# codelion/adaptive-classifier

Measured on NVIDIA H100. Metric: queries/sec predict() bert-base 128-tok, 1M x 768 prototypes, higher is better.
Workload: dtype f16

## Files before the change

### adaptive_classifier_b200/csrc/common.cuh

```cuda
#pragma once

#include <cuda_runtime.h>
#include <cuda.h>
#include <stdint.h>
#include <stdio.h>
#include <string.h>
#include <string>

#include "../../include/adaptive_b200.h"

namespace ac {

void set_error(const char *fmt, ...);
int check_cuda(cudaError_t e, const char *what);

#define AC_CUDA(call)                                                \
    do {                                                             \
        int _rc = ::ac::check_cuda((call), #call);                   \
        if (_rc != 0) return _rc;                                    \
    } while (0)

#define AC_REQUIRE(cond, ...)                                        \
    do {                                                             \
        if (!(cond)) {                                               \
// ... 9 lines not shown
#define AC_LAUNCH_CHECK()                                            \
    do {                                                             \
        ::ac::count_launch();                                        \
        AC_CUDA(cudaGetLastError());                                 \
    } while (0)

enum { PROF_GEMM_LINEAR = 0, PROF_ATTENTION = 1, PROF_KNN_COARSE = 2, PROF_KNN_EXACT = 3, PROF_KNN_PASS2 = 4, PROF_NUM = 5 };
int prof_begin(int cls, double flops, double bytes, cudaStream_t s);
void prof_end(int slot, cudaStream_t s);

static inline size_t align_up(size_t x, size_t a) { return (x + a - 1) / a * a; }
int sm_count();

__device__ __forceinline__ uint32_t smem_u32(const void *p) {
    return static_cast<uint32_t>(__cvta_generic_to_shared(p));
}

__device__ __forceinline__ float round_tf32(float x) {
    uint32_t u = __float_as_uint(x);
    u += 0x0FFFu + ((u >> 13) & 1u);
    u &= 0xFFFFE000u;
    return __uint_as_float(u);
}

__device__ __forceinline__ float warp_sum(float v) {
#pragma unroll
    for (int o = 16; o > 0; o >>= 1) v += __shfl_xor_sync(0xffffffffu, v, o);
    return v;
}
__device__ __forceinline__ float warp_max(float v) {
#pragma unroll
    for (int o = 16; o > 0; o >>= 1) v = fmaxf(v, __shfl_xor_sync(0xffffffffu, v, o));
    return v;
}

__device__ __forceinline__ void mbar_init(uint64_t *bar, uint32_t count) {
    asm volatile("mbarrier.init.shared::cta.b64 [%0], %1;" ::"r"(smem_u32(bar)), "r"(count));
}
__device__ __forceinline__ void fence_mbar_init() {
    asm volatile("fence.mbarrier_init.release.cluster;" ::: "memory");
}
__device__ __forceinline__ void mbar_arrive_expect_tx(uint64_t *bar, uint32_t bytes) {
    asm volatile("mbarrier.arrive.expect_tx.shared::cta.b64 _, [%0], %1;" ::"r"(smem_u32(bar)), "r"(bytes)
                 : "memory");
}
__device__ __forceinline__ void mbar_arrive(uint64_t *bar) {
    asm volatile("mbarrier.arrive.shared::cta.b64 _, [%0];" ::"r"(smem_u32(bar)) : "memory");
}
__device__ __forceinline__ bool mbar_try_wait(uint64_t *bar, uint32_t parity) {
    uint32_t ok;
    asm volatile(
        "{\n\t"
        ".reg .pred p;\n\t"
        "mbarrier.try_wait.parity.shared::cta.b64 p, [%1], %2;\n\t"
        "selp.u32 %0, 1, 0, p;\n\t"
        "}"
        : "=r"(ok)
        : "r"(smem_u32(bar)), "r"(parity)
        : "memory");
    return ok != 0;
}
__device__ __forceinline__ void mbar_wait(uint64_t *bar, uint32_t parity) {
    while (!mbar_try_wait(bar, parity)) {
    }
}

__device__ __forceinline__ void tma_prefetch_desc(const CUtensorMap *m) {
    asm volatile("prefetch.tensormap [%0];" ::"l"(reinterpret_cast<uint64_t>(m)) : "memory");
}
__device__ __forceinline__ void tma_load_2d(void *smem_dst, const CUtensorMap *m, uint64_t *bar, int c0, int c1) {
    asm volatile(
        "cp.async.bulk.tensor.2d.shared::cluster.global.tile.mbarrier::complete_tx::bytes [%0], [%1, {%3, %4}], [%2];"
        ::"r"(smem_u32(smem_dst)), "l"(reinterpret_cast<uint64_t>(m)), "r"(smem_u32(bar)), "r"(c0), "r"(c1)
        : "memory");
}
__device__ __forceinline__ void fence_proxy_async_smem() {
    asm volatile("fence.proxy.async.shared::cta;" ::: "memory");
}

__device__ __forceinline__ void named_bar_sync(int id, int nthreads) {
    asm volatile("bar.sync %0, %1;" ::"r"(id), "r"(nthreads) : "memory");
}

template <int N>
__device__ __forceinline__ void setmaxnreg_inc() { asm volatile("setmaxnreg.inc.sync.aligned.u32 %0;" ::"n"(N)); }
template <int N>
__device__ __forceinline__ void setmaxnreg_dec() { asm volatile("setmaxnreg.dec.sync.aligned.u32 %0;" ::"n"(N)); }

__device__ __forceinline__ uint64_t wgmma_desc_sw128(uint32_t smem_addr) {
    uint64_t d = 0;
    d |= static_cast<uint64_t>((smem_addr & 0x3FFFFu) >> 4);
    d |= static_cast<uint64_t>(1) << 16;
    d |= static_cast<uint64_t>(1024 >> 4) << 32;
    d |= static_cast<uint64_t>(1) << 62;
    return d;
}
__device__ __forceinline__ void wgmma_fence() { asm volatile("wgmma.fence.sync.aligned;" ::: "memory"); }
__device__ __forceinline__ void wgmma_commit() { asm volatile("wgmma.commit_group.sync.aligned;" ::: "memory"); }
template <int N>
__device__ __forceinline__ void wgmma_wait() { asm volatile("wgmma.wait_group.sync.aligned %0;" ::"n"(N) : "memory"); }

__device__ __forceinline__ void wgmma_m64n128_f16(float (&d)[64], uint64_t a_desc, uint64_t b_desc, uint32_t accumulate) {
    asm volatile(
        "{\n\t"
        ".reg .pred p;\n\t"
        "setp.ne.b32 p, %66, 0;\n\t"
        "wgmma.mma_async.sync.aligned.m64n128k16.f32.f16.f16 "
        "{%0, %1, %2, %3, %4, %5, %6, %7, %8, %9, %10, %11, %12, %13, %14, %15, "
        "%16, %17, %18, %19, %20, %21, %22, %23, %24, %25, %26, %27, %28, %29, %30, %31, "
        "%32, %33, %34, %35, %36, %37, %38, %39, %40, %41, %42, %43, %44, %45, %46, %47, "
        "%48, %49, %50, %51, %52, %53, %54, %55, %56, %57, %58, %59, %60, %61, %62, %63}, "
        "%64, %65, p, 1, 1, 0, 0;\n\t"
        "}"
        : "+f"(d[0]), "+f"(d[1]), "+f"(d[2]), "+f"(d[3]), "+f"(d[4]), "+f"(d[5]), "+f"(d[6]), "+f"(d[7]),
          "+f"(d[8]), "+f"(d[9]), "+f"(d[10]), "+f"(d[11]), "+f"(d[12]), "+f"(d[13]), "+f"(d[14]), "+f"(d[15]),
          "+f"(d[16]), "+f"(d[17]), "+f"(d[18]), "+f"(d[19]), "+f"(d[20]), "+f"(d[21]), "+f"(d[22]), "+f"(d[23]),
          "+f"(d[24]), "+f"(d[25]), "+f"(d[26]), "+f"(d[27]), "+f"(d[28]), "+f"(d[29]), "+f"(d[30]), "+f"(d[31]),
          "+f"(d[32]), "+f"(d[33]), "+f"(d[34]), "+f"(d[35]), "+f"(d[36]), "+f"(d[37]), "+f"(d[38]), "+f"(d[39]),
          "+f"(d[40]), "+f"(d[41]), "+f"(d[42]), "+f"(d[43]), "+f"(d[44]), "+f"(d[45]), "+f"(d[46]), "+f"(d[47]),
          "+f"(d[48]), "+f"(d[49]), "+f"(d[50]), "+f"(d[51]), "+f"(d[52]), "+f"(d[53]), "+f"(d[54]), "+f"(d[55]),
          "+f"(d[56]), "+f"(d[57]), "+f"(d[58]), "+f"(d[59]), "+f"(d[60]), "+f"(d[61]), "+f"(d[62]), "+f"(d[63])
        : "l"(a_desc), "l"(b_desc), "r"(accumulate));
}
__device__ __forceinline__ void wgmma_m64n128_tf32(float (&d)[64], uint64_t a_desc, uint64_t b_desc, uint32_t accumulate) {
    asm volatile(
        "{\n\t"
        ".reg .pred p;\n\t"
        "setp.ne.b32 p, %66, 0;\n\t"
        "wgmma.mma_async.sync.aligned.m64n128k8.f32.tf32.tf32 "
        "{%0, %1, %2, %3, %4, %5, %6, %7, %8, %9, %10, %11, %12, %13, %14, %15, "
        "%16, %17, %18, %19, %20, %21, %22, %23, %24, %25, %26, %27, %28, %29, %30, %31, "
        "%32, %33, %34, %35, %36, %37, %38, %39, %40, %41, %42, %43, %44, %45, %46, %47, "
        "%48, %49, %50, %51, %52, %53, %54, %55, %56, %57, %58, %59, %60, %61, %62, %63}, "
        "%64, %65, p, 1, 1;\n\t"
        "}"
        : "+f"(d[0]), "+f"(d[1]), "+f"(d[2]), "+f"(d[3]), "+f"(d[4]), "+f"(d[5]), "+f"(d[6]), "+f"(d[7]),
          "+f"(d[8]), "+f"(d[9]), "+f"(d[10]), "+f"(d[11]), "+f"(d[12]), "+f"(d[13]), "+f"(d[14]), "+f"(d[15]),
          "+f"(d[16]), "+f"(d[17]), "+f"(d[18]), "+f"(d[19]), "+f"(d[20]), "+f"(d[21]), "+f"(d[22]), "+f"(d[23]),
          "+f"(d[24]), "+f"(d[25]), "+f"(d[26]), "+f"(d[27]), "+f"(d[28]), "+f"(d[29]), "+f"(d[30]), "+f"(d[31]),
          "+f"(d[32]), "+f"(d[33]), "+f"(d[34]), "+f"(d[35]), "+f"(d[36]), "+f"(d[37]), "+f"(d[38]), "+f"(d[39]),
          "+f"(d[40]), "+f"(d[41]), "+f"(d[42]), "+f"(d[43]), "+f"(d[44]), "+f"(d[45]), "+f"(d[46]), "+f"(d[47]),
          "+f"(d[48]), "+f"(d[49]), "+f"(d[50]), "+f"(d[51]), "+f"(d[52]), "+f"(d[53]), "+f"(d[54]), "+f"(d[55]),
          "+f"(d[56]), "+f"(d[57]), "+f"(d[58]), "+f"(d[59]), "+f"(d[60]), "+f"(d[61]), "+f"(d[62]), "+f"(d[63])
        : "l"(a_desc), "l"(b_desc), "r"(accumulate));
}
__device__ __forceinline__ void wgmma_m64n64_f16(float (&d)[32], uint64_t a_desc, uint64_t b_desc, uint32_t accumulate) {
    asm volatile(
        "{\n\t"
        ".reg .pred p;\n\t"
        "setp.ne.b32 p, %34, 0;\n\t"
        "wgmma.mma_async.sync.aligned.m64n64k16.f32.f16.f16 "
        "{%0, %1, %2, %3, %4, %5, %6, %7, %8, %9, %10, %11, %12, %13, %14, %15, "
        "%16, %17, %18, %19, %20, %21, %22, %23, %24, %25, %26, %27, %28, %29, %30, %31}, "
        "%32, %33, p, 1, 1, 0, 0;\n\t"
        "}"
        : "+f"(d[0]), "+f"(d[1]), "+f"(d[2]), "+f"(d[3]), "+f"(d[4]), "+f"(d[5]), "+f"(d[6]), "+f"(d[7]),
          "+f"(d[8]), "+f"(d[9]), "+f"(d[10]), "+f"(d[11]), "+f"(d[12]), "+f"(d[13]), "+f"(d[14]), "+f"(d[15]),
          "+f"(d[16]), "+f"(d[17]), "+f"(d[18]), "+f"(d[19]), "+f"(d[20]), "+f"(d[21]), "+f"(d[22]), "+f"(d[23]),
          "+f"(d[24]), "+f"(d[25]), "+f"(d[26]), "+f"(d[27]), "+f"(d[28]), "+f"(d[29]), "+f"(d[30]), "+f"(d[31])
        : "l"(a_desc), "l"(b_desc), "r"(accumulate));
}
__device__ __forceinline__ void wgmma_m64n32_f16(float (&d)[16], uint64_t a_desc, uint64_t b_desc, uint32_t accumulate) {
    asm volatile(
        "{\n\t"
        ".reg .pred p;\n\t"
        "setp.ne.b32 p, %18, 0;\n\t"
// ... 50 lines not shown
```

### adaptive_classifier_b200/csrc/encoder.cu

```cuda
#include "gemm_tc.cuh"
#include <cuda_fp16.h>
#include <math_constants.h>
#include <algorithm>
#include <array>
#include <type_traits>
#include <vector>

namespace ac {

__device__ __forceinline__ float ex2_approx(float x) {
    float y;
    asm("ex2.approx.ftz.f32 %0, %1;" : "=f"(y) : "f"(x));
    return y;
}
__device__ __forceinline__ float rcp_approx(float x) {
    float y;
    asm("rcp.approx.ftz.f32 %0, %1;" : "=f"(y) : "f"(x));
    return y;
}
__device__ __forceinline__ float gelu_erf(float y) {
    const float ay = fabsf(y);
    const float t = rcp_approx(fmaf(0.3275911f * 0.70710678118654752440f, ay, 1.f));
    float p = fmaf(0.5f * 1.061405429f, t, 0.5f * -1.453152027f);
    p = fmaf(p, t, 0.5f * 1.421413741f);
// ... 894 lines not shown
    if (tid == 0) {
        issue(0);
        if (nblk > 1) issue(1);
    }
    score.begin(cta);

    const int qrow = warp * 32 + lane;
    const int qglob = q0 + qrow;
    const float *srow = sS + qrow * ATT_S_LD;
    const float scale_log2 = rsqrtf(static_cast<float>(Score::SCALE_TERMS * DH)) * 1.44269504088896340736f;
    const float sl2 = Score::EX2_ROWS ? 1.f : scale_log2;
    const int frow = 16 * warp + (lane >> 2);
    const uint32_t sp_base = smem_u32(sP);
    float mx = -CUDART_INF_F, sum = 0.f;
    float o[2][DH / 2];
#pragma unroll
    for (int half = 0; half < 2; ++half)
#pragma unroll
        for (int j = 0; j < DH / 2; ++j) o[half][j] = 0.f;

#pragma unroll 1
    for (int i = 0; i < nblk; ++i) {
        const int st = i & 1, key0 = (kb0 + i) * 128;
        mbar_wait_guarded(bar + st, (i >> 1) & 1);
        att_scores<DH>(sQ, sK + st * ATTS_STAGE_BYTES, sS);
        __syncthreads();
        score.add_block_terms(cta, i);

        uint32_t kmask[4];
        att_key_bits(mask, row0, S, key0, qglob, window, lane, kmask);
        float bmx = -CUDART_INF_F;
#pragma unroll
        for (int ci = 0; ci < 4; ++ci) {
            float r[32];
            acc_row_ld32(srow + 32 * ci, r);
            score.row(r, cta, key0 + 32 * ci, scale_log2);
#pragma unroll
            for (int jj = 0; jj < 32; ++jj)
                if ((kmask[ci] >> jj) & 1u) bmx = fmaxf(bmx, r[jj]);
        }
        const float mnew = fmaxf(mx, bmx);
        const float alpha = (mx == -CUDART_INF_F) ? 0.f : ex2_approx((mx - mnew) * sl2);
        const float mxs = (mnew == -CUDART_INF_F) ? 0.f : mnew * sl2;
        float bsum = 0.f;
#pragma unroll
        for (int ci = 0; ci < 4; ++ci) {
            float r[32];
            acc_row_ld32(srow + 32 * ci, r);
            score.row(r, cta, key0 + 32 * ci, scale_log2);
            uint32_t pk[16];
            att_exp_pack(r, kmask[ci], sl2, mxs, bsum, pk);
            att_store_p(sp_base, qrow, 32 * ci, pk);
        }
        sum = fmaf(sum, alpha, bsum);
        mx = mnew;
        sAlpha[qrow] = alpha;
        fence_proxy_async_smem();
        __syncthreads();

#pragma unroll
        for (int half = 0; half < 2; ++half) {
            const float a0 = sAlpha[64 * half + frow], a1 = sAlpha[64 * half + frow + 8];
#pragma unroll
            for (int j = 0; j < DH / 8; ++j) {
                o[half][4 * j] *= a0;
                o[half][4 * j + 1] *= a0;
                o[half][4 * j + 2] *= a1;
                o[half][4 * j + 3] *= a1;
            }
        }
        att_pv<DH>(sP, sVt + st * ATTS_STAGE_BYTES, o, true);
        __syncthreads();
        if (tid == 0 && i + 2 < nblk) issue(i + 2);
        score.after_pv(cta, i);
    }

    wgmma_store_acc(o[0], sS, ATT_S_LD);
    wgmma_store_acc(o[1], sS + 64 * ATT_S_LD, ATT_S_LD);
    __syncthreads();
    const float inv = (sum > 0.f) ? 1.f / sum : 0.f;
    if (qglob < S) att_write_row<DH>(srow, inv, ctx + (row0 + qglob) * H + h * DH);
}

constexpr int ATTL_THREADS = 288;
constexpr int ATTL_STAGES = 4;
constexpr int ATTL_STAGE_BYTES = 32 * 1024;
constexpr int ATTL_OFF_STAGE = 16 * 1024;
constexpr int ATTL_OFF_BITS = ATTL_OFF_STAGE + ATTL_STAGES * ATTL_STAGE_BYTES;
constexpr int ATTL_OFF_BAR = ATTL_OFF_BITS + AC_MODERNBERT_MAX_S / 8;
constexpr int ATTL_SMEM = ATTL_OFF_BAR + (1 + 2 * ATTL_STAGES) * 8 + 1024 ;
static_assert(ATTL_SMEM <= 227 * 1024, "long-attention CTA exceeds the shared-memory limit");

__global__ void __launch_bounds__(ATTL_THREADS, 1)
attention_long_kernel(const __grid_constant__ CUtensorMap tmap_qk, const __grid_constant__ CUtensorMap tmap_vt,
                      const int32_t *__restrict__ mask, int B, int S, int heads, int H, int ,
                      __half *__restrict__ ctx, const __grid_constant__ ScorePlain) {
    extern __shared__ uint8_t smem_raw[];
    uint8_t *smem = reinterpret_cast<uint8_t *>((reinterpret_cast<uintptr_t>(smem_raw) + 1023) & ~uintptr_t(1023));
    uint8_t *sQ = smem;
    uint32_t *sBits = reinterpret_cast<uint32_t *>(smem + ATTL_OFF_BITS);
    uint64_t *bar_q = reinterpret_cast<uint64_t *>(smem + ATTL_OFF_BAR);
    uint64_t *full = bar_q + 1, *empty = full + ATTL_STAGES;

    const int tid = threadIdx.x, warp = tid >> 5, lane = tid & 31;
    const int b = blockIdx.x / heads, h = blockIdx.x % heads;
    const int q0 = blockIdx.y * 128;
    const int row0 = b * S;
    const int nblk = (S + 127) / 128;

    if (tid == 0) {
        tma_prefetch_desc(&tmap_qk);
        tma_prefetch_desc(&tmap_vt);
        mbar_init(bar_q, 1);
        for (int st = 0; st < ATTL_STAGES; ++st) {
            mbar_init(full + st, 1);
            mbar_init(empty + st, 8);
        }
        fence_mbar_init();
    }
    __syncthreads();

    if (warp == 8) {
        if (lane == 0) {
            const int vrow = (b * heads + h) * 64;
            mbar_arrive_expect_tx(bar_q, 16 * 1024);
            tma_load_2d(sQ, &tmap_qk, bar_q, h * 64, row0 + q0);
            for (int i = 0; i < nblk; ++i) {
                const int st = i % ATTL_STAGES, key0 = i * 128;
                if (i >= ATTL_STAGES) mbar_wait_guarded(empty + st, (i / ATTL_STAGES - 1) & 1);
                uint8_t *sK = smem + ATTL_OFF_STAGE + st * ATTL_STAGE_BYTES, *sVt = sK + 16 * 1024;
                mbar_arrive_expect_tx(full + st, ATTL_STAGE_BYTES);
                tma_load_2d(sK, &tmap_qk, full + st, H + h * 64, row0 + key0);
                tma_load_2d(sVt, &tmap_vt, full + st, key0, vrow);
                tma_load_2d(sVt + 8192, &tmap_vt, full + st, key0 + 64, vrow);
            }
        }
        return;
    }

    for (int w = warp; w < 4 * nblk; w += 8) {
        const int key = 32 * w + lane;
        const bool ok = key < S && (!mask || mask[row0 + key] != 0);
        const uint32_t bits = __ballot_sync(0xffffffffu, ok);
        if (lane == 0) sBits[w] = bits;
    }
    named_bar_sync(1, 256);

    const int g = warp >> 2;
    const int r0 = 16 * (warp & 3) + (lane >> 2), c2 = 2 * (lane & 3);
    const float sl2 = 0.125f * 1.44269504088896340736f;
    float o[32];
#pragma unroll
    for (int j = 0; j < 32; ++j) o[j] = 0.f;
    float mx0 = -CUDART_INF_F, mx1 = -CUDART_INF_F, sum0 = 0.f, sum1 = 0.f;
    const uint64_t qa = wgmma_desc_sw128(smem_u32(sQ + g * 8192));
    mbar_wait_guarded(bar_q, 0);

#pragma unroll 1
    for (int i = 0; i < nblk; ++i) {
        const int st = i % ATTL_STAGES;
        const uint8_t *sK = smem + ATTL_OFF_STAGE + st * ATTL_STAGE_BYTES, *sVt = sK + 16 * 1024;
        mbar_wait_guarded(full + st, (i / ATTL_STAGES) & 1);
        float s[64];
        {
            const uint64_t bd = wgmma_desc_sw128(smem_u32(sK));
            wgmma_fence();
#pragma unroll
            for (int k = 0; k < 4; ++k) wgmma_m64n128_f16(s, qa + 2 * k, bd + 2 * k, k != 0);
            wgmma_commit();
            wgmma_wait<0>();
        }
        const uint4 kw = *reinterpret_cast<const uint4 *>(sBits + 4 * i);
        if ((kw.x & kw.y & kw.z & kw.w) != 0xffffffffu) {
            const uint32_t words[4] = {kw.x, kw.y, kw.z, kw.w};
#pragma unroll
            for (int j = 0; j < 16; ++j) {
                const uint32_t bits = words[j >> 2] >> (8 * (j & 3) + c2);
                if (!(bits & 1u)) s[4 * j] = s[4 * j + 2] = -CUDART_INF_F;
                if (!(bits & 2u)) s[4 * j + 1] = s[4 * j + 3] = -CUDART_INF_F;
            }
        }
        float m0 = mx0, m1 = mx1;
#pragma unroll
        for (int j = 0; j < 16; ++j) {
            m0 = fmaxf(m0, fmaxf(s[4 * j], s[4 * j + 1]));
            m1 = fmaxf(m1, fmaxf(s[4 * j + 2], s[4 * j + 3]));
        }
#pragma unroll
        for (int x = 1; x <= 2; x <<= 1) {
            m0 = fmaxf(m0, __shfl_xor_sync(0xffffffffu, m0, x));
            m1 = fmaxf(m1, __shfl_xor_sync(0xffffffffu, m1, x));
        }
        const float alpha0 = (mx0 == -CUDART_INF_F) ? 0.f : ex2_approx((mx0 - m0) * sl2);
        const float alpha1 = (mx1 == -CUDART_INF_F) ? 0.f : ex2_approx((mx1 - m1) * sl2);
        const float ms0 = (m0 == -CUDART_INF_F) ? 0.f : m0 * sl2;
        const float ms1 = (m1 == -CUDART_INF_F) ? 0.f : m1 * sl2;
        mx0 = m0;
        mx1 = m1;
        uint32_t p[32];
        float ps0 = 0.f, ps1 = 0.f;
#pragma unroll
        for (int j = 0; j < 16; ++j) {
            const float e0 = ex2_approx(fmaf(s[4 * j], sl2, -ms0)), e1 = ex2_approx(fmaf(s[4 * j + 1], sl2, -ms0));
            const float e2 = ex2_approx(fmaf(s[4 * j + 2], sl2, -ms1)), e3 = ex2_approx(fmaf(s[4 * j + 3], sl2, -ms1));
            ps0 += e0 + e1;
            ps1 += e2 + e3;
            __half2 h01 = __floats2half2_rn(e0, e1), h23 = __floats2half2_rn(e2, e3);
            p[2 * j] = *reinterpret_cast<uint32_t *>(&h01);
            p[2 * j + 1] = *reinterpret_cast<uint32_t *>(&h23);
        }
        sum0 = fmaf(sum0, alpha0, ps0);
        sum1 = fmaf(sum1, alpha1, ps1);
#pragma unroll
        for (int j = 0; j < 8; ++j) {
            o[4 * j] *= alpha0;
            o[4 * j + 1] *= alpha0;
            o[4 * j + 2] *= alpha1;
            o[4 * j + 3] *= alpha1;
        }
        {
            const uint64_t bv = wgmma_desc_sw128(smem_u32(sVt));
            wgmma_fence();
#pragma unroll
            for (int k = 0; k < 8; ++k) {
                const uint32_t a[4] = {p[4 * k], p[4 * k + 1], p[4 * k + 2], p[4 * k + 3]};
                wgmma_m64n64_f16_rs(o, a, bv + (k >> 2) * 512 + 2 * (k & 3), 1u);
            }
            wgmma_commit();
            wgmma_wait<0>();
        }
        if (lane == 0) mbar_arrive(empty + st);
    }

#pragma unroll
    for (int x = 1; x <= 2; x <<= 1) {
        sum0 += __shfl_xor_sync(0xffffffffu, sum0, x);
        sum1 += __shfl_xor_sync(0xffffffffu, sum1, x);
    }
    const float inv0 = (sum0 > 0.f) ? 1.f / sum0 : 0.f, inv1 = (sum1 > 0.f) ? 1.f / sum1 : 0.f;
    const int q = q0 + 64 * g + r0;
    __half *dst = ctx + (static_cast<int64_t>(row0) + q) * H + h * 64 + c2;
#pragma unroll
    for (int j = 0; j < 8; ++j) {
        if (q < S) *reinterpret_cast<__half2 *>(dst + 8 * j) = __floats2half2_rn(o[4 * j] * inv0, o[4 * j + 1] * inv0);
        if (q + 8 < S)
            *reinterpret_cast<__half2 *>(dst + 8 * static_cast<int64_t>(H) + 8 * j) =
                __floats2half2_rn(o[4 * j + 2] * inv1, o[4 * j + 3] * inv1);
    }
}

__global__ void gather_cls_ln_kernel(const __half *__restrict__ ctx, const float *__restrict__ y, int B, int S, int H,
                                     const float *__restrict__ g, const float *__restrict__ b, float eps,
                                     __half *__restrict__ ctx_cls, float *__restrict__ x_cls) {
    const int bq = blockIdx.x * (blockDim.x >> 5) + (threadIdx.x >> 5);
    const int lane = threadIdx.x & 31;
    if (bq >= B) return;
    const int64_t src = static_cast<int64_t>(bq) * S * H, dst = static_cast<int64_t>(bq) * H;
    for (int i = lane; i < H / 8; i += 32)
        reinterpret_cast<uint4 *>(ctx_cls + dst)[i] = reinterpret_cast<const uint4 *>(ctx + src)[i];
    const int nv = H / 128;
    float4 x[LN_MAXV];
#pragma unroll
    for (int i = 0; i < LN_MAXV; ++i)
        if (i < nv) x[i] = *reinterpret_cast<const float4 *>(y + src + (lane + 32 * i) * 4);
    ln_row(x, nv, H, g, b, eps, lane, x_cls + dst, nullptr);
}

__global__ void pos_gather_kernel(const float *__restrict__ pos_key, const float *__restrict__ pos_query,
                                  const int32_t *__restrict__ rel_index, int span, int heads, int H, __half *__restrict__ out) {
    const int64_t row = static_cast<int64_t>(blockIdx.x) * 4 + (threadIdx.x >> 6);
    const int col = threadIdx.x & 63;
    const int t = static_cast<int>(row % 256), term = static_cast<int>((row / 256) % 2);
    const int h = static_cast<int>((row / 512) % heads);
    const int64_t ld = row / (512 * static_cast<int64_t>(heads));
    const int d = static_cast<int>(ld % ATTS_POS_DELTAS);
    const int64_t l = ld / ATTS_POS_DELTAS;
    float v = 0.f;
    if (t < 255) {
        const int delta = 128 * (d - ATTS_POS_DELTAS / 2);
        const int r = term ? delta + 127 - t : delta + t - 127;
        const int c = min(max(rel_index[AC_ENCODER_MAX_S - 1 + r], 0), 2 * span - 1);
        v = (term ? pos_query : pos_key)[(l * 2 * span + c) * H + 64 * h + col];
    }
    out[row * 64 + col] = __float2half_rn(v);
}

}

using namespace ac;

struct Layer {
    __half *wqkv = nullptr, *wo = nullptr, *w1 = nullptr, *w2 = nullptr;
    CUtensorMap m_wqkv, m_wo, m_w1, m_w2;
    float *c1qkv = nullptr, *c0qkv = nullptr, *c1f = nullptr, *c0f = nullptr;
    float *bo = nullptr, *b2 = nullptr;
    float *ln_ffn_w = nullptr, *ln_ffn_b = nullptr;
    float *ln_out_w = nullptr, *ln_out_b = nullptr;
    int window = 0;
};

struct ac_encoder {
    ac_encoder_config cfg;
    float *word = nullptr, *pos = nullptr, *type = nullptr, *emb_ln_w = nullptr, *emb_ln_b = nullptr;
    __half *emb_proj_w = nullptr;
    float *emb_proj_b = nullptr;
    CUtensorMap m_emb, m_emb_proj;
    std::vector<Layer> layers;
    __half *w1_last = nullptr;
    float *b1_last = nullptr;
    float *x = nullptr, *tmp = nullptr;
    __half *xh = nullptr, *qk = nullptr, *vT = nullptr, *ctx = nullptr, *ffn = nullptr;
    size_t T = 0;
    size_t vt_elems = 0;
    size_t Bc = 0;
    float *x_cls = nullptr, *tmp_cls = nullptr;
    __half *xh_cls = nullptr, *ctx_cls = nullptr, *ffn_cls = nullptr;
    CUtensorMap m_xh_cls, m_ctx_cls, m_ffn_cls;
    CUtensorMap m_xh, m_ctx, m_ffn, m_qk_att, m_vt_att;
    int vt_B = -1, vt_S = -1;
    CUtensorMap p_w1_last;
    float2 *stats_a = nullptr, *stats_b = nullptr, *stats_id = nullptr, *parts = nullptr;
    float *ones = nullptr, *zeros = nullptr;
    float *rope[2] = {nullptr, nullptr};
    float *rel_bias = nullptr;
    __half *pos_g = nullptr;
    CUtensorMap m_pos;
    std::vector<void *> allocs;
    int last_B = 0, last_S = 0;
    bool last_cls_only = false;
};

static int launch_cls_normalize(const float *x, int B, int S, int H, float *out, cudaStream_t s) {
    const int wpb = 8;
    cls_normalize_kernel<<<(B + wpb - 1) / wpb, wpb * 32, 0, s>>>(x, B, S, H, out);
    AC_LAUNCH_CHECK();
    return AC_OK;
}

struct AttVariant { const void *kernel; int smem, threads; };
enum { ATT_PLAIN64, ATT_PLAIN32, ATT_RELBIAS, ATTS_PLAIN64, ATTS_PLAIN32, ATTS_RELBIAS, ATTS_DISENT, ATTL_PLAIN64, ATT_VARIANTS };
static const AttVariant att_variants[ATT_VARIANTS] = {
    {reinterpret_cast<const void *>(attention_kernel<64, ScorePlain>), ATT_SMEM<ScorePlain>, ATT_THREADS},
    {reinterpret_cast<const void *>(attention_kernel<32, ScorePlain>), ATT_SMEM<ScorePlain>, ATT_THREADS},
    {reinterpret_cast<const void *>(attention_kernel<64, ScoreRelBias>), ATT_SMEM<ScoreRelBias>, ATT_THREADS},
    {reinterpret_cast<const void *>(attention_stream_kernel<64, ScorePlain>), ATTS_SMEM<ScorePlain>, ATT_THREADS},
    {reinterpret_cast<const void *>(attention_stream_kernel<32, ScorePlain>), ATTS_SMEM<ScorePlain>, ATT_THREADS},
    {reinterpret_cast<const void *>(attention_stream_kernel<64, ScoreRelBias>), ATTS_SMEM<ScoreRelBias>, ATT_THREADS},
    {reinterpret_cast<const void *>(attention_stream_kernel<64, ScoreDisent>), ATTS_SMEM<ScoreDisent>, ATT_THREADS},
    {reinterpret_cast<const void *>(attention_long_kernel), ATTL_SMEM, ATTL_THREADS},
};

static int launch_attention(ac_encoder *e, const int32_t *mask, int B, int S, int window, bool cls_rows, int layer,
                            cudaStream_t s) {
    const ac_encoder_config &c = e->cfg;
    int H = c.hidden, heads = c.heads;
    const int dh = H / heads;
    AC_REQUIRE(S <= AC_ENCODER_MAX_S || dh == 64, "attention: S=%d > %d needs head_dim 64 (ModernBERT)", S, AC_ENCODER_MAX_S);
    static bool att_attr[64] = {};
    int dev = 0;
    AC_CUDA(cudaGetDevice(&dev));
    if (dev < 0 || dev >= 64 || !att_attr[dev]) {
        for (const AttVariant &v : att_variants)
            AC_CUDA(cudaFuncSetAttribute(v.kernel, cudaFuncAttributeMaxDynamicSharedMemorySize, v.smem));
        if (dev >= 0 && dev < 64) att_attr[dev] = true;
    }
    const int q_blocks = cls_rows ? 1 : (S + 127) / 128;
    const int nq = std::min(S, 128 * q_blocks);
    double keys = 0.0;
    if (window > 0) {
        for (int q = 0; q < nq; ++q) keys += std::min(S - 1, q + window) - std::max(0, q - window) + 1;
    } else {
        keys = static_cast<double>(nq) * S;
    }
    const int slot = prof_begin(PROF_ATTENTION, 4.0 * B * c.heads * keys * dh, 0.0, s);
    const bool streamed = e->pos_g || S > 128;
    ScorePlain plain;
    ScoreRelBias bias;
    ScoreDisent disent;
    void *score = &plain;
    int id = dh == 32 ? (streamed ? ATTS_PLAIN32 : ATT_PLAIN32) : (streamed ? ATTS_PLAIN64 : ATT_PLAIN64);
    if (e->pos_g) {
        disent.tmap_pos = e->m_pos;
        disent.pos_row0 = layer * ATTS_POS_DELTAS * heads * 2 * 256;
        score = &disent;
        id = ATTS_DISENT;
    } else if (e->rel_bias) {
        bias.rel_bias = e->rel_bias;
        score = &bias;
        id = streamed ? ATTS_RELBIAS : ATT_RELBIAS;
    } else if (S > AC_ENCODER_MAX_S && c.arch != AC_ARCH_MODERNBERT) {
        id = ATTL_PLAIN64;
    }
    const AttVariant &v = att_variants[id];
    void *args[] = {&e->m_qk_att, &e->m_vt_att, &mask, &B, &S, &heads, &H, &window, &e->ctx, score};
    cudaLaunchKernel(v.kernel, dim3(B * heads, streamed ? q_blocks : 1), dim3(v.threads), args, v.smem, s);
    prof_end(slot, s);
    AC_LAUNCH_CHECK();
    return AC_OK;
}

template <class T>
static int dev_alloc(ac_encoder *e, T **p, size_t elems) {
    void *q = nullptr;
    AC_CUDA(cudaMalloc(&q, elems * sizeof(T)));
    e->allocs.push_back(q);
    *p = static_cast<T *>(q);
    return AC_OK;
}

static int pack_f32(ac_encoder *e, float **dst, const float *src, size_t n) {
    int rc = dev_alloc(e, dst, n);
    if (rc) return rc;
    round_copy_kernel<<<256, 256>>>(src, *dst, static_cast<int64_t>(n), 0);
    AC_LAUNCH_CHECK();
    return AC_OK;
}
static int pack_f16(ac_encoder *e, __half **dst, const float *src, size_t n) {
    int rc = dev_alloc(e, dst, n);
    if (rc) return rc;
    to_half_kernel<<<256, 256>>>(src, *dst, static_cast<int64_t>(n));
    AC_LAUNCH_CHECK();
    return AC_OK;
}

extern "C" int ac_encoder_destroy(ac_encoder *enc) {
    if (!enc) return AC_OK;
    for (void *p : enc->allocs) cudaFree(p);
    delete enc;
    return AC_OK;
}

static int pack_consumer(ac_encoder *e, int n, const float *const *W, const float *const *bias, const float *gamma,
                         const float *beta, int N, int K, int glu, __half **wp, float **c1, float **c0) {
    const size_t NK = static_cast<size_t>(N) * K;
    int rc;
    if ((rc = dev_alloc(e, wp, n * NK)) || (rc = dev_alloc(e, c1, static_cast<size_t>(n) * N)) ||
        (rc = dev_alloc(e, c0, static_cast<size_t>(n) * N)))
        return rc;
    for (int j = 0; j < n; ++j) {
        pack_defer_kernel<<<(N + 7) / 8, 256>>>(W[j], bias ? bias[j] : nullptr, gamma, beta, N, K, *wp + j * NK, *c1 + j * N,
                                                *c0 + j * N, glu);
        if ((rc = check_cuda(cudaGetLastError(), "pack_defer_kernel"))) return rc;
    }
    return AC_OK;
}

extern "C" int ac_encoder_create(const ac_encoder_config *cfg, const ac_encoder_weights *w, ac_encoder **out) {
    AC_REQUIRE(cfg && w && out, "ac_encoder_create: null argument");
    const bool mb = cfg->arch == AC_ARCH_MODERNBERT;
    AC_REQUIRE(!mb || (cfg->max_pos >= AC_ENCODER_MAX_S && cfg->max_pos <= AC_MODERNBERT_MAX_S && cfg->layer_sliding &&
                       cfg->sliding_window > 0 && cfg->rope_full && cfg->rope_sliding && w->wqkv && w->wi && w->final_norm_w &&
                       (cfg->layers == 1 || w->attn_norm_w)),
               "ac_encoder_create: ModernBERT needs %d <= max_pos <= %d (max_pos=%d), layer_sliding, sliding_window > 0, both "
               "RoPE tables, wqkv, wi, final_norm_w and attn_norm_w", AC_ENCODER_MAX_S, AC_MODERNBERT_MAX_S, cfg->max_pos);
    const bool rot = cfg->arch == AC_ARCH_ROTARY;
    AC_REQUIRE(!rot || (cfg->rope_full && cfg->max_pos >= AC_ENCODER_MAX_S && cfg->max_pos <= AC_MODERNBERT_MAX_S),
               "ac_encoder_create: AC_ARCH_ROTARY needs rope_full and %d <= max_pos <= %d (max_pos=%d)", AC_ENCODER_MAX_S,
               AC_MODERNBERT_MAX_S, cfg->max_pos);
    AC_REQUIRE(cfg->precision == AC_PREC_F16, "ac_encoder_create: only AC_PREC_F16 (fp16 operands, fp32 accumulate) is implemented");
    AC_REQUIRE(cfg->hidden % 128 == 0 && cfg->hidden <= 1024, "ac_encoder_create: hidden=%d must be a multiple of 128, <= 1024", cfg->hidden);
    AC_REQUIRE(cfg->heads > 0 && cfg->hidden % cfg->heads == 0 &&
                   (cfg->hidden / cfg->heads == 64 || (!mb && !rot && cfg->hidden / cfg->heads == 32)),
               "ac_encoder_create: head_dim must be %s (hidden=%d heads=%d)",
               mb ? "64 for ModernBERT" : rot ? "64 for AC_ARCH_ROTARY" : "64 or 32", cfg->hidden, cfg->heads);
    const bool mp = cfg->arch == AC_ARCH_MPNET;
    AC_REQUIRE(!mp || (cfg->rel_bias && cfg->hidden == 64 * cfg->heads),
               "ac_encoder_create: MPNet needs rel_bias and head_dim 64 (hidden=%d heads=%d)", cfg->hidden, cfg->heads);
    const bool db = cfg->arch == AC_ARCH_DEBERTA;
    AC_REQUIRE(!db || (cfg->pos_key && cfg->pos_query && cfg->rel_index && cfg->pos_span > 0 &&
                       cfg->hidden == 64 * cfg->heads),
               "ac_encoder_create: DeBERTa needs pos_key, pos_query, rel_index, pos_span > 0 (pos_span=%d) and head_dim 64 "
               "(hidden=%d heads=%d)", cfg->pos_span, cfg->hidden, cfg->heads);
    AC_REQUIRE(cfg->intermediate % 64 == 0 && cfg->layers > 0 && cfg->max_tokens > 0, "ac_encoder_create: bad dims");
    AC_REQUIRE(cfg->ffn_act == AC_FFN_GELU_ERF || cfg->ffn_act == AC_FFN_GELU_TANH || cfg->ffn_act == AC_FFN_SWIGLU,
               "ac_encoder_create: unknown ffn_act=%d", cfg->ffn_act);
    const bool swiglu = cfg->ffn_act == AC_FFN_SWIGLU;
    AC_REQUIRE(!swiglu || rot, "ac_encoder_create: ffn_act=%d (AC_FFN_SWIGLU) is implemented for AC_ARCH_ROTARY only (arch=%d)",
               cfg->ffn_act, cfg->arch);
// ... 413 lines not shown
```

Before: 17860.

## Replace long-attention kernel with persistent register-softmax kernel for all BERT head-64 attention

```diff
diff --git a/adaptive_classifier_b200/csrc/common.cuh b/adaptive_classifier_b200/csrc/common.cuh
--- a/adaptive_classifier_b200/csrc/common.cuh
+++ b/adaptive_classifier_b200/csrc/common.cuh
@@ -115,6 +115,10 @@
     asm volatile("bar.sync %0, %1;" ::"r"(id), "r"(nthreads) : "memory");
 }
 
+__device__ __forceinline__ void named_bar_arrive(int id, int nthreads) {
+    asm volatile("bar.arrive %0, %1;" ::"r"(id), "r"(nthreads) : "memory");
+}
+
 template <int N>
 __device__ __forceinline__ void setmaxnreg_inc() { asm volatile("setmaxnreg.inc.sync.aligned.u32 %0;" ::"n"(N)); }
 template <int N>
diff --git a/adaptive_classifier_b200/csrc/encoder.cu b/adaptive_classifier_b200/csrc/encoder.cu
--- a/adaptive_classifier_b200/csrc/encoder.cu
+++ b/adaptive_classifier_b200/csrc/encoder.cu
@@ -1000,37 +1000,42 @@
     if (qglob < S) att_write_row<DH>(srow, inv, ctx + (row0 + qglob) * H + h * DH);
 }
 
-constexpr int ATTL_THREADS = 288;
-constexpr int ATTL_STAGES = 4;
-constexpr int ATTL_STAGE_BYTES = 32 * 1024;
-constexpr int ATTL_OFF_STAGE = 16 * 1024;
-constexpr int ATTL_OFF_BITS = ATTL_OFF_STAGE + ATTL_STAGES * ATTL_STAGE_BYTES;
-constexpr int ATTL_OFF_BAR = ATTL_OFF_BITS + AC_MODERNBERT_MAX_S / 8;
-constexpr int ATTL_SMEM = ATTL_OFF_BAR + (1 + 2 * ATTL_STAGES) * 8 + 1024 ;
-static_assert(ATTL_SMEM <= 227 * 1024, "long-attention CTA exceeds the shared-memory limit");
-
-__global__ void __launch_bounds__(ATTL_THREADS, 1)
-attention_long_kernel(const __grid_constant__ CUtensorMap tmap_qk, const __grid_constant__ CUtensorMap tmap_vt,
-                      const int32_t *__restrict__ mask, int B, int S, int heads, int H, int ,
-                      __half *__restrict__ ctx, const __grid_constant__ ScorePlain) {
+constexpr int ATTR_THREADS = 288;
+constexpr int ATTR_STAGES = 4;
+constexpr int ATTR_QSLOTS = 3;
+constexpr int ATTR_STAGE_BYTES = 32 * 1024;
+constexpr int ATTR_BITS_WORDS = AC_MODERNBERT_MAX_S / 32;
+constexpr int ATTR_OFF_STAGE = ATTR_QSLOTS * 16 * 1024;
+constexpr int ATTR_SUM_LD = 4 * 16 + 4;
+constexpr int ATTR_OFF_SUM = ATTR_OFF_STAGE + ATTR_STAGES * ATTR_STAGE_BYTES;
+constexpr int ATTR_OFF_BITS = ATTR_OFF_SUM + 8 * 16 * ATTR_SUM_LD * 4;
+constexpr int ATTR_OFF_BAR = ATTR_OFF_BITS + ATTR_QSLOTS * ATTR_BITS_WORDS * 4;
+constexpr int ATTR_SMEM = ATTR_OFF_BAR + 2 * (ATTR_QSLOTS + ATTR_STAGES) * 8 + 1024 ;
+static_assert(ATTR_SMEM <= 227 * 1024, "register-softmax attention CTA exceeds the shared-memory limit");
+
+__global__ void __launch_bounds__(ATTR_THREADS, 1)
+attention_reg_kernel(const __grid_constant__ CUtensorMap tmap_qk, const __grid_constant__ CUtensorMap tmap_vt,
+                     const int32_t *__restrict__ mask, int B, int S, int heads, int H, int ,
+                     __half *__restrict__ ctx, int q_blocks) {
     extern __shared__ uint8_t smem_raw[];
     uint8_t *smem = reinterpret_cast<uint8_t *>((reinterpret_cast<uintptr_t>(smem_raw) + 1023) & ~uintptr_t(1023));
-    uint8_t *sQ = smem;
-    uint32_t *sBits = reinterpret_cast<uint32_t *>(smem + ATTL_OFF_BITS);
-    uint64_t *bar_q = reinterpret_cast<uint64_t *>(smem + ATTL_OFF_BAR);
-    uint64_t *full = bar_q + 1, *empty = full + ATTL_STAGES;
+    uint32_t *sBits = reinterpret_cast<uint32_t *>(smem + ATTR_OFF_BITS);
+    uint64_t *q_full = reinterpret_cast<uint64_t *>(smem + ATTR_OFF_BAR);
+    uint64_t *q_empty = q_full + ATTR_QSLOTS, *full = q_empty + ATTR_QSLOTS, *empty = full + ATTR_STAGES;
 
     const int tid = threadIdx.x, warp = tid >> 5, lane = tid & 31;
-    const int b = blockIdx.x / heads, h = blockIdx.x % heads;
-    const int q0 = blockIdx.y * 128;
-    const int row0 = b * S;
     const int nblk = (S + 127) / 128;
+    const int items = B * heads * q_blocks;
+    const int my_items = (items - static_cast<int>(blockIdx.x) + static_cast<int>(gridDim.x) - 1) / static_cast<int>(gridDim.x);
 
     if (tid == 0) {
         tma_prefetch_desc(&tmap_qk);
         tma_prefetch_desc(&tmap_vt);
-        mbar_init(bar_q, 1);
-        for (int st = 0; st < ATTL_STAGES; ++st) {
+        for (int s = 0; s < ATTR_QSLOTS; ++s) {
+            mbar_init(q_full + s, 1);
+            mbar_init(q_empty + s, 8);
+        }
+        for (int st = 0; st < ATTR_STAGES; ++st) {
             mbar_init(full + st, 1);
             mbar_init(empty + st, 8);
         }
@@ -1039,104 +1044,140 @@
     __syncthreads();
 
     if (warp == 8) {
-        if (lane == 0) {
-            const int vrow = (b * heads + h) * 64;
-            mbar_arrive_expect_tx(bar_q, 16 * 1024);
-            tma_load_2d(sQ, &tmap_qk, bar_q, h * 64, row0 + q0);
-            for (int i = 0; i < nblk; ++i) {
-                const int st = i % ATTL_STAGES, key0 = i * 128;
-                if (i >= ATTL_STAGES) mbar_wait_guarded(empty + st, (i / ATTL_STAGES - 1) & 1);
-                uint8_t *sK = smem + ATTL_OFF_STAGE + st * ATTL_STAGE_BYTES, *sVt = sK + 16 * 1024;
-                mbar_arrive_expect_tx(full + st, ATTL_STAGE_BYTES);
-                tma_load_2d(sK, &tmap_qk, full + st, H + h * 64, row0 + key0);
-                tma_load_2d(sVt, &tmap_vt, full + st, key0, vrow);
-                tma_load_2d(sVt + 8192, &tmap_vt, full + st, key0 + 64, vrow);
-            }
+        int kv = 0;
+        for (int it = 0; it < my_items; ++it) {
+            const int item = static_cast<int>(blockIdx.x) + it * static_cast<int>(gridDim.x);
+            const int bh = item / q_blocks, q0 = (item % q_blocks) * 128;
+            const int b = bh / heads, h = bh % heads, row0 = b * S;
+            const int qs = it % ATTR_QSLOTS;
+            if (it >= ATTR_QSLOTS) mbar_wait_guarded(q_empty + qs, (it / ATTR_QSLOTS - 1) & 1);
+            uint32_t *bits = sBits + qs * ATTR_BITS_WORDS;
+            for (int w0 = 0; w0 < 4 * nblk; w0 += 32) {
+                bool ok[32];
+#pragma unroll
+                for (int j = 0; j < 32; ++j) {
+                    const int key = 32 * (w0 + j) + lane;
+                    ok[j] = key < S && (!mask || mask[row0 + key] != 0);
+                }
+#pragma unroll
+                for (int j = 0; j < 32; ++j) {
+                    const uint32_t m = __ballot_sync(0xffffffffu, ok[j]);
+                    if (lane == 0) bits[w0 + j] = m;
+                }
+            }
+            if (lane == 0) {
+                mbar_arrive_expect_tx(q_full + qs, 16 * 1024);
+                tma_load_2d(smem + qs * 16 * 1024, &tmap_qk, q_full + qs, h * 64, row0 + q0);
+                const int vrow = (b * heads + h) * 64;
+                for (int i = 0; i < nblk; ++i, ++kv) {
+                    const int st = kv % ATTR_STAGES, key0 = i * 128;
+                    if (kv >= ATTR_STAGES) mbar_wait_guarded(empty + st, (kv / ATTR_STAGES - 1) & 1);
+                    uint8_t *sK = smem + ATTR_OFF_STAGE + st * ATTR_STAGE_BYTES, *sVt = sK + 16 * 1024;
+                    mbar_arrive_expect_tx(full + st, ATTR_STAGE_BYTES);
+                    tma_load_2d(sK, &tmap_qk, full + st, H + h * 64, row0 + key0);
+                    tma_load_2d(sVt, &tmap_vt, full + st, key0, vrow);
+                    tma_load_2d(sVt + 8192, &tmap_vt, full + st, key0 + 64, vrow);
+                }
+            }
+            __syncwarp();
         }
         return;
     }
-
-    for (int w = warp; w < 4 * nblk; w += 8) {
-        const int key = 32 * w + lane;
-        const bool ok = key < S && (!mask || mask[row0 + key] != 0);
-        const uint32_t bits = __ballot_sync(0xffffffffu, ok);
-        if (lane == 0) sBits[w] = bits;
-    }
-    named_bar_sync(1, 256);
 
     const int g = warp >> 2;
     const int r0 = 16 * (warp & 3) + (lane >> 2), c2 = 2 * (lane & 3);
-    const float sl2 = 0.125f * 1.44269504088896340736f;
-    float o[32];
-#pragma unroll
-    for (int j = 0; j < 32; ++j) o[j] = 0.f;
-    float mx0 = -CUDART_INF_F, mx1 = -CUDART_INF_F, sum0 = 0.f, sum1 = 0.f;
-    const uint64_t qa = wgmma_desc_sw128(smem_u32(sQ + g * 8192));
-    mbar_wait_guarded(bar_q, 0);
-
+    const float sl2 = rsqrtf(static_cast<float>(64)) * 1.44269504088896340736f;
+    float *wsum = reinterpret_cast<float *>(smem + ATTR_OFF_SUM) + warp * 16 * ATTR_SUM_LD;
+    float *pair_a = wsum + (lane >> 2) * ATTR_SUM_LD + 16 * (lane & 3), *pair_b = pair_a + 8 * ATTR_SUM_LD;
+    if (g == 1) named_bar_arrive(1, 256);
+    int kv = 0;
 #pragma unroll 1
-    for (int i = 0; i < nblk; ++i) {
-        const int st = i % ATTL_STAGES;
-        const uint8_t *sK = smem + ATTL_OFF_STAGE + st * ATTL_STAGE_BYTES, *sVt = sK + 16 * 1024;
-        mbar_wait_guarded(full + st, (i / ATTL_STAGES) & 1);
-        float s[64];
-        {
-            const uint64_t bd = wgmma_desc_sw128(smem_u32(sK));
-            wgmma_fence();
-#pragma unroll
-            for (int k = 0; k < 4; ++k) wgmma_m64n128_f16(s, qa + 2 * k, bd + 2 * k, k != 0);
-            wgmma_commit();
-            wgmma_wait<0>();
-        }
-        const uint4 kw = *reinterpret_cast<const uint4 *>(sBits + 4 * i);
-        if ((kw.x & kw.y & kw.z & kw.w) != 0xffffffffu) {
-            const uint32_t words[4] = {kw.x, kw.y, kw.z, kw.w};
+    for (int it = 0; it < my_items; ++it) {
+        const int item = static_cast<int>(blockIdx.x) + it * static_cast<int>(gridDim.x);
+        const int bh = item / q_blocks, q0 = (item % q_blocks) * 128;
+        const int b = bh / heads, h = bh % heads, row0 = b * S;
+        const int qs = it % ATTR_QSLOTS;
+        const uint64_t qa = wgmma_desc_sw128(smem_u32(smem + qs * 16 * 1024 + g * 8192));
+        const uint32_t *bits = sBits + qs * ATTR_BITS_WORDS;
+        float o[32];
+#pragma unroll
+        for (int j = 0; j < 32; ++j) o[j] = 0.f;
+        float mx0 = -CUDART_INF_F, mx1 = -CUDART_INF_F, sum0 = 0.f, sum1 = 0.f;
+        mbar_wait_guarded(q_full + qs, (it / ATTR_QSLOTS) & 1);
+
+#pragma unroll 1
+        for (int i = 0; i < nblk; ++i, ++kv) {
+            const int st = kv % ATTR_STAGES;
+            const uint8_t *sK = smem + ATTR_OFF_STAGE + st * ATTR_STAGE_BYTES, *sVt = sK + 16 * 1024;
+            mbar_wait_guarded(full + st, (kv / ATTR_STAGES) & 1);
+            named_bar_sync(1 + g, 256);
+            float s[64];
+            {
+                const uint64_t bd = wgmma_desc_sw128(smem_u32(sK));
+                wgmma_fence();
+#pragma unroll
+                for (int k = 0; k < 4; ++k) wgmma_m64n128_f16(s, qa + 2 * k, bd + 2 * k, k != 0);
+                wgmma_commit();
+                wgmma_wait<0>();
+            }
+            const uint4 kw = *reinterpret_cast<const uint4 *>(bits + 4 * i);
+            if (i == nblk - 1) {
+                __syncwarp();
+                if (lane == 0) mbar_arrive(q_empty + qs);
+            }
+            if ((kw.x & kw.y & kw.z & kw.w) != 0xffffffffu) {
+                const uint32_t words[4] = {kw.x, kw.y, kw.z, kw.w};
+#pragma unroll
+                for (int j = 0; j < 16; ++j) {
+                    const uint32_t kb = words[j >> 2] >> (8 * (j & 3) + c2);
+                    if (!(kb & 1u)) s[4 * j] = s[4 * j + 2] = -CUDART_INF_F;
+                    if (!(kb & 2u)) s[4 * j + 1] = s[4 * j + 3] = -CUDART_INF_F;
+                }
+            }
+            float m0 = mx0, m1 = mx1;
 #pragma unroll
             for (int j = 0; j < 16; ++j) {
-                const uint32_t bits = words[j >> 2] >> (8 * (j & 3) + c2);
-                if (!(bits & 1u)) s[4 * j] = s[4 * j + 2] = -CUDART_INF_F;
-                if (!(bits & 2u)) s[4 * j + 1] = s[4 * j + 3] = -CUDART_INF_F;
-            }
-        }
-        float m0 = mx0, m1 = mx1;
-#pragma unroll
-        for (int j = 0; j < 16; ++j) {
-            m0 = fmaxf(m0, fmaxf(s[4 * j], s[4 * j + 1]));
-            m1 = fmaxf(m1, fmaxf(s[4 * j + 2], s[4 * j + 3]));
-        }
-#pragma unroll
-        for (int x = 1; x <= 2; x <<= 1) {
-            m0 = fmaxf(m0, __shfl_xor_sync(0xffffffffu, m0, x));
-            m1 = fmaxf(m1, __shfl_xor_sync(0xffffffffu, m1, x));
-        }
-        const float alpha0 = (mx0 == -CUDART_INF_F) ? 0.f : ex2_approx((mx0 - m0) * sl2);
-        const float alpha1 = (mx1 == -CUDART_INF_F) ? 0.f : ex2_approx((mx1 - m1) * sl2);
-        const float ms0 = (m0 == -CUDART_INF_F) ? 0.f : m0 * sl2;
-        const float ms1 = (m1 == -CUDART_INF_F) ? 0.f : m1 * sl2;
-        mx0 = m0;
-        mx1 = m1;
-        uint32_t p[32];
-        float ps0 = 0.f, ps1 = 0.f;
-#pragma unroll
-        for (int j = 0; j < 16; ++j) {
-            const float e0 = ex2_approx(fmaf(s[4 * j], sl2, -ms0)), e1 = ex2_approx(fmaf(s[4 * j + 1], sl2, -ms0));
-            const float e2 = ex2_approx(fmaf(s[4 * j + 2], sl2, -ms1)), e3 = ex2_approx(fmaf(s[4 * j + 3], sl2, -ms1));
-            ps0 += e0 + e1;
-            ps1 += e2 + e3;
-            __half2 h01 = __floats2half2_rn(e0, e1), h23 = __floats2half2_rn(e2, e3);
-            p[2 * j] = *reinterpret_cast<uint32_t *>(&h01);
-            p[2 * j + 1] = *reinterpret_cast<uint32_t *>(&h23);
-        }
-        sum0 = fmaf(sum0, alpha0, ps0);
-        sum1 = fmaf(sum1, alpha1, ps1);
-#pragma unroll
-        for (int j = 0; j < 8; ++j) {
-            o[4 * j] *= alpha0;
-            o[4 * j + 1] *= alpha0;
-            o[4 * j + 2] *= alpha1;
-            o[4 * j + 3] *= alpha1;
-        }
-        {
+                m0 = fmaxf(m0, fmaxf(s[4 * j], s[4 * j + 1]));
+                m1 = fmaxf(m1, fmaxf(s[4 * j + 2], s[4 * j + 3]));
+            }
+#pragma unroll
+            for (int x = 1; x <= 2; x <<= 1) {
+                m0 = fmaxf(m0, __shfl_xor_sync(0xffffffffu, m0, x));
+                m1 = fmaxf(m1, __shfl_xor_sync(0xffffffffu, m1, x));
+            }
+            const float alpha0 = (mx0 == -CUDART_INF_F) ? 0.f : ex2_approx((mx0 - m0) * sl2);
+            const float alpha1 = (mx1 == -CUDART_INF_F) ? 0.f : ex2_approx((mx1 - m1) * sl2);
+            const float ms0 = (m0 == -CUDART_INF_F) ? 0.f : m0 * sl2;
+            const float ms1 = (m1 == -CUDART_INF_F) ? 0.f : m1 * sl2;
+            mx0 = m0;
+            mx1 = m1;
+            uint32_t p[32];
+#pragma unroll
+            for (int q4 = 0; q4 < 4; ++q4) {
+                float pa[4], pb[4];
+#pragma unroll
+                for (int jj = 0; jj < 4; ++jj) {
+                    const int j = 4 * q4 + jj;
+                    const float e0 = ex2_approx(fmaf(s[4 * j], sl2, -ms0)), e1 = ex2_approx(fmaf(s[4 * j + 1], sl2, -ms0));
+                    const float e2 = ex2_approx(fmaf(s[4 * j + 2], sl2, -ms1)), e3 = ex2_approx(fmaf(s[4 * j + 3], sl2, -ms1));
+                    pa[jj] = e0 + e1;
+                    pb[jj] = e2 + e3;
+                    __half2 h01 = __floats2half2_rn(e0, e1), h23 = __floats2half2_rn(e2, e3);
+                    p[2 * j] = *reinterpret_cast<uint32_t *>(&h01);
+                    p[2 * j + 1] = *reinterpret_cast<uint32_t *>(&h23);
+                }
+                *reinterpret_cast<float4 *>(pair_a + 4 * q4) = make_float4(pa[0], pa[1], pa[2], pa[3]);
+                *reinterpret_cast<float4 *>(pair_b + 4 * q4) = make_float4(pb[0], pb[1], pb[2], pb[3]);
+            }
+            __syncwarp();
+            named_bar_arrive(1 + (g ^ 1), 256);
+#pragma unroll
+            for (int j = 0; j < 8; ++j) {
+                o[4 * j] *= alpha0;
+                o[4 * j + 1] *= alpha0;
+                o[4 * j + 2] *= alpha1;
+                o[4 * j + 3] *= alpha1;
+            }
             const uint64_t bv = wgmma_desc_sw128(smem_u32(sVt));
             wgmma_fence();
 #pragma unroll
@@ -1145,26 +1186,43 @@
                 wgmma_m64n64_f16_rs(o, a, bv + (k >> 2) * 512 + 2 * (k & 3), 1u);
             }
             wgmma_commit();
+            float bsum = 0.f;
+            if (lane < 16) {
+                const float *row = wsum + lane * ATTR_SUM_LD;
+#pragma unroll
+                for (int q4 = 0; q4 < 4; ++q4) {
+                    float4 v[4];
+#pragma unroll
+                    for (int t = 0; t < 4; ++t) v[t] = *reinterpret_cast<const float4 *>(row + 16 * t + 4 * q4);
+#pragma unroll
+                    for (int t = 0; t < 4; ++t) bsum += v[t].x;
+#pragma unroll
+                    for (int t = 0; t < 4; ++t) bsum += v[t].y;
+#pragma unroll
+                    for (int t = 0; t < 4; ++t) bsum += v[t].z;
+#pragma unroll
+                    for (int t = 0; t < 4; ++t) bsum += v[t].w;
+                }
+            }
+            sum0 = fmaf(sum0, alpha0, __shfl_sync(0xffffffffu, bsum, lane >> 2));
+            sum1 = fmaf(sum1, alpha1, __shfl_sync(0xffffffffu, bsum, (lane >> 2) + 8));
+            __syncwarp();
             wgmma_wait<0>();
-        }
-        if (lane == 0) mbar_arrive(empty + st);
-    }
-
-#pragma unroll
-    for (int x = 1; x <= 2; x <<= 1) {
-        sum0 += __shfl_xor_sync(0xffffffffu, sum0, x);
-        sum1 += __shfl_xor_sync(0xffffffffu, sum1, x);
-    }
-    const float inv0 = (sum0 > 0.f) ? 1.f / sum0 : 0.f, inv1 = (sum1 > 0.f) ? 1.f / sum1 : 0.f;
-    const int q = q0 + 64 * g + r0;
-    __half *dst = ctx + (static_cast<int64_t>(row0) + q) * H + h * 64 + c2;
-#pragma unroll
-    for (int j = 0; j < 8; ++j) {
-        if (q < S) *reinterpret_cast<__half2 *>(dst + 8 * j) = __floats2half2_rn(o[4 * j] * inv0, o[4 * j + 1] * inv0);
-        if (q + 8 < S)
-            *reinterpret_cast<__half2 *>(dst + 8 * static_cast<int64_t>(H) + 8 * j) =
-                __floats2half2_rn(o[4 * j + 2] * inv1, o[4 * j + 3] * inv1);
-    }
+            if (lane == 0) mbar_arrive(empty + st);
+        }
+
+        const float inv0 = (sum0 > 0.f) ? 1.f / sum0 : 0.f, inv1 = (sum1 > 0.f) ? 1.f / sum1 : 0.f;
+        const int q = q0 + 64 * g + r0;
+        __half *dst = ctx + (static_cast<int64_t>(row0) + q) * H + h * 64 + c2;
+#pragma unroll
+        for (int j = 0; j < 8; ++j) {
+            if (q < S) *reinterpret_cast<__half2 *>(dst + 8 * j) = __floats2half2_rn(o[4 * j] * inv0, o[4 * j + 1] * inv0);
+            if (q + 8 < S)
+                *reinterpret_cast<__half2 *>(dst + 8 * static_cast<int64_t>(H) + 8 * j) =
+                    __floats2half2_rn(o[4 * j + 2] * inv1, o[4 * j + 3] * inv1);
+        }
+    }
+    if (g == 0) named_bar_sync(1, 256);
 }
 
 __global__ void gather_cls_ln_kernel(const __half *__restrict__ ctx, const float *__restrict__ y, int B, int S, int H,
@@ -1255,17 +1313,24 @@
     return AC_OK;
 }
 
-struct AttVariant { const void *kernel; int smem, threads; };
-enum { ATT_PLAIN64, ATT_PLAIN32, ATT_RELBIAS, ATTS_PLAIN64, ATTS_PLAIN32, ATTS_RELBIAS, ATTS_DISENT, ATTL_PLAIN64, ATT_VARIANTS };
+enum AttGrid {
+    GRID_SEQ_HEAD,
+    GRID_QBLOCK,
+    GRID_PERSISTENT,
+};
+struct AttVariant { const void *kernel; int smem, threads; AttGrid grid; };
+enum { ATT_PLAIN64, ATT_PLAIN32, ATT_RELBIAS, ATTS_PLAIN64, ATTS_PLAIN32, ATTS_RELBIAS, ATTS_DISENT, ATTR_PLAIN64, ATT_VARIANTS };
 static const AttVariant att_variants[ATT_VARIANTS] = {
-    {reinterpret_cast<const void *>(attention_kernel<64, ScorePlain>), ATT_SMEM<ScorePlain>, ATT_THREADS},
-    {reinterpret_cast<const void *>(attention_kernel<32, ScorePlain>), ATT_SMEM<ScorePlain>, ATT_THREADS},
-    {reinterpret_cast<const void *>(attention_kernel<64, ScoreRelBias>), ATT_SMEM<ScoreRelBias>, ATT_THREADS},
-    {reinterpret_cast<const void *>(attention_stream_kernel<64, ScorePlain>), ATTS_SMEM<ScorePlain>, ATT_THREADS},
-    {reinterpret_cast<const void *>(attention_stream_kernel<32, ScorePlain>), ATTS_SMEM<ScorePlain>, ATT_THREADS},
-    {reinterpret_cast<const void *>(attention_stream_kernel<64, ScoreRelBias>), ATTS_SMEM<ScoreRelBias>, ATT_THREADS},
-    {reinterpret_cast<const void *>(attention_stream_kernel<64, ScoreDisent>), ATTS_SMEM<ScoreDisent>, ATT_THREADS},
-    {reinterpret_cast<const void *>(attention_long_kernel), ATTL_SMEM, ATTL_THREADS},
+    {reinterpret_cast<const void *>(attention_kernel<64, ScorePlain>), ATT_SMEM<ScorePlain>, ATT_THREADS, GRID_SEQ_HEAD},
+    {reinterpret_cast<const void *>(attention_kernel<32, ScorePlain>), ATT_SMEM<ScorePlain>, ATT_THREADS, GRID_SEQ_HEAD},
+    {reinterpret_cast<const void *>(attention_kernel<64, ScoreRelBias>), ATT_SMEM<ScoreRelBias>, ATT_THREADS, GRID_SEQ_HEAD},
+    {reinterpret_cast<const void *>(attention_stream_kernel<64, ScorePlain>), ATTS_SMEM<ScorePlain>, ATT_THREADS, GRID_QBLOCK},
+    {reinterpret_cast<const void *>(attention_stream_kernel<32, ScorePlain>), ATTS_SMEM<ScorePlain>, ATT_THREADS, GRID_QBLOCK},
+    {reinterpret_cast<const void *>(attention_stream_kernel<64, ScoreRelBias>), ATTS_SMEM<ScoreRelBias>, ATT_THREADS,
+     GRID_QBLOCK},
+    {reinterpret_cast<const void *>(attention_stream_kernel<64, ScoreDisent>), ATTS_SMEM<ScoreDisent>, ATT_THREADS,
+     GRID_QBLOCK},
+    {reinterpret_cast<const void *>(attention_reg_kernel), ATTR_SMEM, ATTR_THREADS, GRID_PERSISTENT},
 };
 
 static int launch_attention(ac_encoder *e, const int32_t *mask, int B, int S, int window, bool cls_rows, int layer,
@@ -1282,7 +1347,7 @@
             AC_CUDA(cudaFuncSetAttribute(v.kernel, cudaFuncAttributeMaxDynamicSharedMemorySize, v.smem));
         if (dev >= 0 && dev < 64) att_attr[dev] = true;
     }
-    const int q_blocks = cls_rows ? 1 : (S + 127) / 128;
+    int q_blocks = cls_rows ? 1 : (S + 127) / 128;
     const int nq = std::min(S, 128 * q_blocks);
     double keys = 0.0;
     if (window > 0) {
@@ -1306,12 +1371,17 @@
         bias.rel_bias = e->rel_bias;
         score = &bias;
         id = streamed ? ATTS_RELBIAS : ATT_RELBIAS;
-    } else if (S > AC_ENCODER_MAX_S && c.arch != AC_ARCH_MODERNBERT) {
-        id = ATTL_PLAIN64;
+    } else if (dh == 64 && window == 0 && c.arch != AC_ARCH_MODERNBERT) {
+        score = &q_blocks;
+        id = ATTR_PLAIN64;
     }
     const AttVariant &v = att_variants[id];
+    const int items = B * heads * q_blocks;
+    const dim3 grid = v.grid == GRID_PERSISTENT ? dim3(std::min(items, sm_count()))
+                      : v.grid == GRID_QBLOCK   ? dim3(B * heads, q_blocks)
+                                                : dim3(B * heads);
     void *args[] = {&e->m_qk_att, &e->m_vt_att, &mask, &B, &S, &heads, &H, &window, &e->ctx, score};
-    cudaLaunchKernel(v.kernel, dim3(B * heads, streamed ? q_blocks : 1), dim3(v.threads), args, v.smem, s);
+    cudaLaunchKernel(v.kernel, grid, dim3(v.threads), args, v.smem, s);
     prof_end(slot, s);
     AC_LAUNCH_CHECK();
     return AC_OK;
```

Measured after the change: 18090, median of 6. Within noise of the previous version (+1.3%).
